# AutonomousVehicleLaboratory/vision_semantic_segmentation

Measured on AMD Instinct MI355X. Metric: fused frames/sec/GPU (1920x1080 + 120k pts) + max|dlog-odds| vs ref, higher is better.
Workload: dtype f16 hi+lo split, MX-FP4 correction passes, fp32 accumulate

## Files before the change

### vision_semantic_segmentation_amd/csrc/seg_dwpw.hip

```cpp
#include "seg_types.h"

namespace avl {
namespace {

constexpr int TM = 128;
constexpr int TN = 256;
constexpr int A_STAGE = TM * 128;
constexpr int W_STAGE = TN * 128;
constexpr int LDS_W = 0, LDS_A = 2 * W_STAGE, LDS_P = LDS_A + 2 * A_STAGE;
constexpr int P_STEP = 8 * 6 * 8 * 4;

struct DwPwArgs {
    const void* X;
    const void* X_lo;
    const void* Wc;
    const float* bc;
    float* LG;
    unsigned char* labels;
    int ncls;
    int tiles_x;
    const void* W;
    const float* bias;
    const uint32_t* dwp;
    const int* order;
// ... 189 lines not shown
                if constexpr (WSUB != 1) {
                    if (p.C_lo) {
#pragma unroll
                        for (int i = 0; i < 8; ++i) { lo[i] -= (float)(HT)lo[i]; hi[i] -= (float)(HT)hi[i]; }
                        HT* cl = static_cast<HT*>(p.C_lo) + (long long)m * p.ldc + nbase;
                        Vec8<HT>::store(cl, lo);
                        Vec8<HT>::store(cl + 8, hi);
                    }
                }
            }
        }
    }
}

constexpr int X_LDS_W = 0, X_LDS_AH = 2 * W_STAGE, X_LDS_AL = X_LDS_AH + 2 * A_STAGE, X_LDS_P = X_LDS_AL + A_STAGE;
constexpr int XP_RING = 4;
constexpr int FP_STEP = 8 * 10 * 8 * 4;

__global__ void __launch_bounds__(512) k_dwpw_x(DwPwArgs p) {
    constexpr int PSTEP = FP_STEP;
    typedef f16 HT;
    typedef typename Half16<HT>::v8 v8;
    extern __shared__ __attribute__((aligned(16))) char lds[];
    const int tid = threadIdx.x, lane = tid & 63;
    const int wave = __builtin_amdgcn_readfirstlane(tid >> 6);
    const int wm = wave >> 2, wn = wave & 3;
    const int nt = blockIdx.x % p.ntiles;
    const int bm = blockIdx.x / p.ntiles, slot = (bm & 7) * p.per_xcd + (bm >> 3);
    if (slot >= p.mtiles) return;
    dwpw_image(p);
    const int mt = p.order[slot];
    const int nk = p.K / 64;

    const uint4* psrc = reinterpret_cast<const uint4*>(p.dwp);
    uint4 pnext = make_uint4(0u, 0u, 0u, 0u);
    auto load_p = [&](int s) { if (tid < PSTEP / 16 && s < nk) pnext = psrc[s * (PSTEP / 16) + tid]; };
    auto store_p = [&](int s) { if (tid < PSTEP / 16 && s < nk) *reinterpret_cast<uint4*>(lds + X_LDS_P + (s & (XP_RING - 1)) * PSTEP + tid * 16) = pnext; };
    for (int s = 0; s < 3; ++s) { load_p(s); store_p(s); }

    const int chunk = tid & 7, r0 = tid >> 3;
    unsigned voff[2][9];
#pragma unroll
    for (int q = 0; q < 2; ++q) {
        const int m = mt * TM + r0 + q * 64;
        const int y = m / p.OW, x = m - y * p.OW;
#pragma unroll
        for (int t = 0; t < 9; ++t) {
            const int iy = y - p.pad + (t / 3) * p.dil, ix = x - p.pad + (t % 3) * p.dil;
            const bool ok = m < p.M && iy >= 0 && iy < p.H && ix >= 0 && ix < p.Wd;
            voff[q][t] = ok ? (unsigned)(((long long)iy * p.Wd + ix) * p.ldx + chunk * 8) * 2u : 0x7fffff00u;
        }
    }
    const int wchunk = tid & 7, wrow0 = tid >> 3;
    const __amdgpu_buffer_rsrc_t wrsrc = __builtin_amdgcn_make_buffer_rsrc(
        const_cast<char*>(static_cast<const char*>(p.W) + (long long)nt * TN * p.K * 4), 0, TN * p.K * 4, 0x00020000);
    int w_voff[4];
#pragma unroll
    for (int i = 0; i < 4; ++i) w_voff[i] = (wrow0 + 64 * i) * p.K * 4 + wchunk * 16;
    v4i wl[4];
    auto load_w = [&](int h) {
#pragma unroll
        for (int i = 0; i < 4; ++i) wl[i] = __builtin_amdgcn_raw_buffer_load_b128(wrsrc, w_voff[i], h * 128, 0);
    };
    auto store_w = [&](int h) {
#pragma unroll
        for (int i = 0; i < 4; ++i) {
            const int r = wrow0 + 64 * i;
            const int key = ((r >> 1) & 1) | (((r >> 4) & 3) << 1);
            *reinterpret_cast<v4i*>(lds + X_LDS_W + (h & 1) * W_STAGE + r * 128 + ((wchunk ^ key) << 4)) = wl[i];
        }
    };

    const int fr = lane & 15, kq = lane >> 4;
    int a_off[4], w_off[4], a_key[4], w_key[4];
#pragma unroll
    for (int mi = 0; mi < 4; ++mi) {
        const int row = wm * 64 + mi * 16 + fr;
        a_off[mi] = row * 128;
        a_key[mi] = row & 7;
    }
#pragma unroll
    for (int nj = 0; nj < 4; ++nj) {
        const int row = wn * 64 + (fr >> 2) * 16 + nj * 4 + (fr & 3);
        w_off[nj] = X_LDS_W + row * 128;
        w_key[nj] = ((row >> 1) & 1) | (((row >> 4) & 3) << 1);
    }
    f32x4 acc[4][4];
    {
        const int nb = nt * TN + wn * 64 + kq * 16;
#pragma unroll
        for (int nj = 0; nj < 4; ++nj) {
            const float4 b = *reinterpret_cast<const float4*>(p.bias + nb + 4 * nj);
#pragma unroll
            for (int mi = 0; mi < 4; ++mi) acc[mi][nj] = f32x4{b.x, b.y, b.z, b.w};
        }
    }

    v4i raw[2][9];
    const __amdgpu_buffer_rsrc_t xrsrc = __builtin_amdgcn_make_buffer_rsrc(const_cast<void*>(p.X), 0, (int)p.x_bytes, 0x00020000);
    auto load_taps = [&](int s, int q) {
#pragma unroll
        for (int t = 0; t < 9; ++t) raw[q][t] = __builtin_amdgcn_raw_buffer_load_b128(xrsrc, (int)voff[q][t], s * 128, 0);
    };
// ... 1 lines not shown
    auto produce_a = [&](int s, int q) {
        float o[8];
        const float* pf = reinterpret_cast<const float*>(lds + X_LDS_P + (s & (XP_RING - 1)) * PSTEP + chunk * (10 * 8 * 4));
        {
            const float4 b0 = *reinterpret_cast<const float4*>(pf + 9 * 8), b1 = *reinterpret_cast<const float4*>(pf + 9 * 8 + 4);
            o[0] = b0.x; o[1] = b0.y; o[2] = b0.z; o[3] = b0.w;
            o[4] = b1.x; o[5] = b1.y; o[6] = b1.z; o[7] = b1.w;
        }
        typedef _Float16 h2 __attribute__((ext_vector_type(2)));
#pragma unroll
        for (int t = 0; t < 9; ++t) {
            const float4 w0 = *reinterpret_cast<const float4*>(pf + t * 8), w1 = *reinterpret_cast<const float4*>(pf + t * 8 + 4);
            const float wt[8] = {w0.x, w0.y, w0.z, w0.w, w1.x, w1.y, w1.z, w1.w};
#pragma unroll
            for (int j = 0; j < 4; ++j) {
                const int u = raw[q][t][j];
                const h2 v = __builtin_bit_cast(h2, u);
                o[2 * j] = __builtin_fmaf((float)v[0], wt[2 * j], o[2 * j]);
                o[2 * j + 1] = __builtin_fmaf((float)v[1], wt[2 * j + 1], o[2 * j + 1]);
            }
        }
        float ol[8];
#pragma unroll
        for (int i = 0; i < 8; ++i) {
            o[i] = fmaxf(o[i], 0.f);
            ol[i] = o[i] - (float)(HT)o[i];
        }
        const int row = r0 + q * 64;
        const int sw = row * 128 + ((chunk ^ (row & 7)) << 4);
        Vec8<HT>::store(reinterpret_cast<HT*>(lds + X_LDS_AH + (s & 1) * A_STAGE + sw), o);
        Vec8<HT>::store(reinterpret_cast<HT*>(lds + X_LDS_AL + sw), ol);
    };

    load_taps(0, 0);
    load_taps(0, 1);
    load_w(0);
    __syncthreads();
    produce_a(0, 0);
    produce_a(0, 1);
    store_w(0);
    if (nk > 1) { load_taps(1, 0); load_taps(1, 1); }

    for (int s = 0; s < nk; ++s) {
        const bool more = s + 1 < nk, more2 = s + 2 < nk;
        asm volatile("s_waitcnt lgkmcnt(0)" ::: "memory");
        __builtin_amdgcn_s_barrier();
        load_w(2 * s + 1);
        load_p(s + 3);
#pragma unroll
        for (int kk = 0; kk < 2; ++kk) {
            v8 wa[4], ah[4], al[4];
#pragma unroll
            for (int nj = 0; nj < 4; ++nj) wa[nj] = *reinterpret_cast<const v8*>(lds + w_off[nj] + (((kk * 4 + kq) ^ w_key[nj]) << 4));
#pragma unroll
            for (int mi = 0; mi < 4; ++mi) {
                ah[mi] = *reinterpret_cast<const v8*>(lds + X_LDS_AH + (s & 1) * A_STAGE + a_off[mi] + (((kk * 4 + kq) ^ a_key[mi]) << 4));
                al[mi] = *reinterpret_cast<const v8*>(lds + X_LDS_AL + a_off[mi] + (((kk * 4 + kq) ^ a_key[mi]) << 4));
            }
#pragma unroll
            for (int mi = 0; mi < 4; ++mi)
#pragma unroll
                for (int nj = 0; nj < 4; ++nj) acc[mi][nj] = Half16<HT>::mfma(wa[nj], al[mi], acc[mi][nj]);
#pragma unroll
            for (int mi = 0; mi < 4; ++mi)
#pragma unroll
                for (int nj = 0; nj < 4; ++nj) acc[mi][nj] = Half16<HT>::mfma(wa[nj], ah[mi], acc[mi][nj]);
        }
        store_w(2 * s + 1);
        store_p(s + 3);
        asm volatile("s_waitcnt lgkmcnt(0)" ::: "memory");
        __builtin_amdgcn_s_barrier();
        if (more) load_w(2 * s + 2);
#pragma unroll
        for (int kk = 0; kk < 2; ++kk) {
            v8 wa[4], ah[4];
#pragma unroll
            for (int nj = 0; nj < 4; ++nj) wa[nj] = *reinterpret_cast<const v8*>(lds + W_STAGE + w_off[nj] + (((kk * 4 + kq) ^ w_key[nj]) << 4));
#pragma unroll
            for (int mi = 0; mi < 4; ++mi)
                ah[mi] = *reinterpret_cast<const v8*>(lds + X_LDS_AH + (s & 1) * A_STAGE + a_off[mi] + (((kk * 4 + kq) ^ a_key[mi]) << 4));
#pragma unroll
            for (int mi = 0; mi < 4; ++mi)
#pragma unroll
                for (int nj = 0; nj < 4; ++nj) acc[mi][nj] = Half16<HT>::mfma(wa[nj], ah[mi], acc[mi][nj]);
            if (more) {
                produce_a(s + 1, kk);
                if (more2) load_taps(s + 2, kk);
            }
        }
        if (more) store_w(2 * s + 2);
    }

    const int nbase = nt * TN + wn * 64 + kq * 16;
    if (nbase + 16 <= p.N) {
#pragma unroll
        for (int mi = 0; mi < 4; ++mi) {
            const int m = mt * TM + wm * 64 + mi * 16 + fr;
            if (m < p.M) {
                float lo[8], hi[8];
#pragma unroll
                for (int nj = 0; nj < 2; ++nj)
#pragma unroll
                    for (int r = 0; r < 4; ++r) {
                        lo[nj * 4 + r] = fmaxf(acc[mi][nj][r], 0.f);
                        hi[nj * 4 + r] = fmaxf(acc[mi][2 + nj][r], 0.f);
                    }
                HT* cp = static_cast<HT*>(p.C) + (long long)m * p.ldc + nbase;
                Vec8<HT>::store(cp, lo);
                Vec8<HT>::store(cp + 8, hi);
                if (p.C_lo) {
#pragma unroll
                    for (int i = 0; i < 8; ++i) { lo[i] -= (float)(HT)lo[i]; hi[i] -= (float)(HT)hi[i]; }
                    HT* cl = static_cast<HT*>(p.C_lo) + (long long)m * p.ldc + nbase;
                    Vec8<HT>::store(cl, lo);
                    Vec8<HT>::store(cl + 8, hi);
                }
            }
        }
    }
}

int launch_dwpw_x(const DwPwArgs& a, hipStream_t s) {
    constexpr int lds_bytes = X_LDS_P + XP_RING * FP_STEP;
    static_assert(lds_bytes <= 160 * 1024, "k_dwpw_x LDS");
// ... 409 lines not shown
```

### vision_semantic_segmentation_amd/csrc/seg_gconv_mfma.hip

```cpp
#include <cstring>

#include "seg_types.h"

namespace avl {
namespace {

constexpr int TW = 32;
constexpr int CC = 64;

template <typename HT>
struct GconvArgs {
    const HT* in;
    const HT* in_lo;
    const HT* w;
    const float* bias;
    HT* out;
    HT* out_lo;
    char* oq[2];
    char* os[2];
    long long o_srows;
    int H, W, in_ld, OH, OW, out_ld, C;
    int stride, dil;
    int th;
    int tiles_x, tiles_y, cchunks;
    int comb;
    int nsp, nslots;
    int walk;
    int tile_bytes;
    int tw_magic;
    const char* w4;
    const char* w4s;
    const char* xq[2];
    const char* xs[2];
    long long x_srows;
    int dephase;
};

constexpr int ROWS_PITCH = 40, ROWS_IN_TH = 6;
constexpr int ROWS_TILE_BYTES = ROWS_IN_TH * ROWS_PITCH * 128 + 4 * 4096 + 2 * 1024;
static_assert(2 * ROWS_TILE_BYTES <= 160 * 1024 && ROWS_PITCH % 8 == 0 && ROWS_PITCH >= TW + 2, "two row-aligned tile buffers fit the CU's LDS");

template <typename T>
__device__ __forceinline__ T lds_load(unsigned byte_addr) {
    return *(const __attribute__((address_space(3))) T*)(size_t)byte_addr;
}

template <typename HT, int WS, int NJ, bool XS = false, bool ROWS = false>
__global__ void __launch_bounds__(512) k_gconv_mfma(GconvArgs<HT> p) {
    static_assert(!XS || WS == 1, "a split input goes with split weights");
    static_assert(!ROWS || (WS == 2 && NJ == 2), "the row-aligned tile is the MX variant's four-row tile");
    typedef typename Half16<HT>::v8 v8;
    extern __shared__ __attribute__((aligned(16))) char lds[];
    const int tid = threadIdx.x, lane = tid & 63;
    const int wave = __builtin_amdgcn_readfirstlane(tid >> 6);
    {
        const long long ipix = (long long)p.H * p.W, opix = (long long)p.OH * p.OW;
        p.in = image_base(p.in, ipix, p.in_ld);
        p.in_lo = image_base(p.in_lo, ipix, p.in_ld);
        p.out = image_base(p.out, opix, p.out_ld);
        p.out_lo = image_base(p.out_lo, opix, p.out_ld);
#pragma unroll
        for (int pl = 0; pl < 2; ++pl) {
            p.oq[pl] = image_base(p.oq[pl], opix, p.C / 2);
            p.os[pl] = image_base(p.os[pl], opix, 8);
            p.xq[pl] = image_base(p.xq[pl], ipix, p.C / 2);
            p.xs[pl] = image_base(p.xs[pl], ipix, 8);
        }
    }
    int bid = blockIdx.x;
    {
        const int nwg = gridDim.x, xcd = bid & 7, local = bid >> 3, q = nwg >> 3, r = nwg & 7;
        bid = (xcd < r ? xcd * (q + 1) : r * (q + 1) + (xcd - r) * q) + local;
    }
    const int cchunk = bid % p.cchunks, slot = bid / p.cchunks;
    const int s = ROWS ? 1 : p.stride;
    const int d = ROWS ? 1 : p.comb ? 1 : p.dil;
    const int step = p.comb ? p.dil : 1;
    const int th = ROWS ? 4 : p.th;
    const int in_th = ROWS ? ROWS_IN_TH : (th - 1) * s + 2 * d + 1, in_tw = ROWS ? ROWS_PITCH : (TW - 1) * s + 2 * d + 1;
    const int tile_bytes = ROWS ? ROWS_TILE_BYTES : p.tile_bytes;
    const int c0 = cchunk * CC;
    const int npix = in_th * in_tw;
    const int ngroups = (npix + 7) >> 3;
    const unsigned lds0 = lds_addr(lds);
    const int n64 = (npix + 63) >> 6;
    const int QBASE = ngroups * 1024, QT = n64 * 1024, SBASE = QBASE + 4 * QT, ST = n64 * 256;
    const bool has_lo = WS == 2 && p.xq[1] != nullptr;
    const int LOBASE = ngroups * 1024;
// ... 18 lines not shown
            const int cy = min(max(iy, 0), p.H - 1), cx = min(max(ix, 0), p.W - 1);
            const unsigned voff = ((unsigned)(cy * p.W + cx) * (unsigned)p.in_ld + ((cphys ^ (pix & 7)) << 3)) * (unsigned)sizeof(HT);
            glds16_saddr(p.in + c0, voff, lds0 + buf * tile_bytes + gi * 1024);
            if constexpr (XS) glds16_saddr(p.in_lo + c0, voff, lds0 + buf * tile_bytes + LOBASE + gi * 1024);
            oob |= outside << it;
        }
        if constexpr (WS == 2) {
            const int pwbits = has_lo ? 2 : 1;
            it = 16;
            for (int item = wave; item < (n64 << pwbits); item += 8, ++it) {
                const int pw = item & ((1 << pwbits) - 1), gq = item >> pwbits, w = pw & 1, pl = pw >> 1;
                const int pix = gq * 64 + lane;
                const int ly = (pix * p.tw_magic) >> 16, lx = pix - ly * in_tw;
                const int iy = iy0 + ly * step, ix = ix0 + lx * step;
                const unsigned outside = (unsigned)(pix >= npix) | (unsigned)((unsigned)iy >= (unsigned)p.H) | (unsigned)((unsigned)ix >= (unsigned)p.W);
                const int cy = min(max(iy, 0), p.H - 1), cx = min(max(ix, 0), p.W - 1);
                glds16_saddr(xq0 + pl * xq_delta + c0 / 2 + w * 16, (unsigned)(cy * p.W + cx) * (unsigned)(p.C / 2),
                             lds0 + buf * tile_bytes + QBASE + (pl * 2 + w) * QT + gq * 1024);
                oob |= outside << it;
            }
            for (int item = wave; item < (n64 << (pwbits - 1)); item += 8) {
                const int pl = item & ((1 << (pwbits - 1)) - 1), gq = item >> (pwbits - 1);
                const int pix = gq * 64 + lane;
                const int ly = (pix * p.tw_magic) >> 16, lx = pix - ly * in_tw;
                const int cy = min(max(iy0 + ly * step, 0), p.H - 1), cx = min(max(ix0 + lx * step, 0), p.W - 1);
                glds4_saddr(xs0 + pl * xs_delta + ((long long)(c0 >> 8) * p.x_srows) * 8 + ((c0 >> 5) & 4), (unsigned)(cy * p.W + cx) * 8u,
                            lds0 + buf * tile_bytes + SBASE + pl * ST + gq * 256);
            }
        }
        return oob;
    };
    const int col_lane = (lane >> 3) * step;
    const unsigned swz_lane = (unsigned)(((lane & 7) ^ (lane >> 3)) << 3) * (unsigned)sizeof(HT);
    auto stage_rows = [&](int ty, int tx, int ry, int rx, int buf) -> unsigned {
        const int iy0 = ry + (ty * 4 - 1) * step, ix0 = rx + (tx * TW - 1) * step;
        const unsigned dst = lds0 + buf * ROWS_TILE_BYTES;
        const unsigned ld_bytes = (unsigned)p.in_ld * (unsigned)sizeof(HT);
        unsigned oob = 0;
#pragma unroll
        for (int it = 0; it < 4; ++it) {
            const int gi = wave + 8 * it;
            if (gi < ROWS_IN_TH * (ROWS_PITCH / 8)) {
                const int ly = gi / (ROWS_PITCH / 8), g8 = gi - ly * (ROWS_PITCH / 8);
                const int iy = iy0 + ly * step, ix = ix0 + g8 * 8 * step + col_lane;
                const unsigned outside = (unsigned)((unsigned)iy >= (unsigned)p.H) | (unsigned)((unsigned)ix >= (unsigned)p.W);
                const int cy = min(max(iy, 0), p.H - 1), cx = min(max(ix, 0), p.W - 1);
                const unsigned voff = (unsigned)(cy * p.W) * ld_bytes + __umul24((unsigned)cx, ld_bytes) + swz_lane;
                glds16_saddr(p.in + c0, voff, dst + gi * 1024);
                oob |= outside << it;
            }
        }
        const int pwbits = has_lo ? 2 : 1;
        int it = 16;
        for (int item = wave; item < (4 << pwbits); item += 8, ++it) {
            const int pw = item & ((1 << pwbits) - 1), gq = item >> pwbits, w = pw & 1, pl = pw >> 1;
            const int pix = gq * 64 + lane;
            const int ly = (pix * 1639) >> 16, lx = pix - ly * ROWS_PITCH;
            const int iy = __mul24(ly, step) + iy0, ix = __mul24(lx, step) + ix0;
            const unsigned outside = (unsigned)(pix >= ROWS_IN_TH * ROWS_PITCH) | (unsigned)((unsigned)iy >= (unsigned)p.H) | (unsigned)((unsigned)ix >= (unsigned)p.W);
            const int cy = min(max(iy, 0), p.H - 1), cx = min(max(ix, 0), p.W - 1);
            glds16_saddr(xq0 + pl * xq_delta + c0 / 2 + w * 16, (__umul24((unsigned)cy, (unsigned)p.W) + (unsigned)cx) * (unsigned)(p.C / 2),
                         dst + QBASE + (pl * 2 + w) * QT + gq * 1024);
            oob |= outside << it;
        }
        for (int item = wave; item < (4 << (pwbits - 1)); item += 8) {
            const int pl = item & ((1 << (pwbits - 1)) - 1), gq = item >> (pwbits - 1);
            const int pix = gq * 64 + lane;
            const int ly = (pix * 1639) >> 16, lx = pix - ly * ROWS_PITCH;
            const int cy = min(max(__mul24(ly, step) + iy0, 0), p.H - 1), cx = min(max(__mul24(lx, step) + ix0, 0), p.W - 1);
            glds4_saddr(xs0 + pl * xs_delta + ((long long)(c0 >> 8) * p.x_srows) * 8 + ((c0 >> 5) & 4), (__umul24((unsigned)cy, (unsigned)p.W) + (unsigned)cx) * 8u,
                        dst + SBASE + pl * ST + gq * 256);
        }
        return oob;
    };
    const int per = (p.nsp + p.nslots - 1) / p.nslots;
    const int sp_step = ROWS || p.walk ? 1 : p.nslots, sp_end = ROWS || p.walk ? min(p.nsp, (slot + 1) * per) : p.nsp;
    int sp = ROWS || p.walk ? slot * per : slot, buf = 0;
    int ty = 0, tx = 0, ry = 0, rx = 0, nty = 0, ntx = 0, nry = 0, nrx = 0;
    auto advance = [&](int& y, int& x, int& cy, int& cx) {
        if (++y == p.tiles_y) {
            y = 0;
            if (++x == p.tiles_x) {
                x = 0;
                if (++cx == p.dil) { cx = 0; ++cy; }
            }
        }
    };
    if constexpr (ROWS) {
        ty = sp % p.tiles_y;
        const int r1 = sp / p.tiles_y;
        tx = r1 % p.tiles_x;
        const int cmb = r1 / p.tiles_x;
        ry = p.comb ? cmb / p.dil : 0; rx = p.comb ? cmb % p.dil : 0;
        nty = ty; ntx = tx; nry = ry; nrx = rx;
        advance(nty, ntx, nry, nrx);
    }
    auto stage_tile = [&](bool next, int b) -> unsigned {
        if constexpr (ROWS) return next ? stage_rows(nty, ntx, nry, nrx, b) : stage_rows(ty, tx, ry, rx, b);
        else return stage(next ? sp + sp_step : sp, b);
    };
    unsigned oob = sp < sp_end ? stage_tile(false, 0) : 0u;

    const int win = wave & 1;
    const int part = wave >> 1;
    const int fr = lane & 15, kq = lane >> 4;
    constexpr int NT = WS == 1 ? 18 : 9;
    v8 wf[2][NT];
    {
        const HT* wp = p.w + (long long)(cchunk * 2 + win) * (2 * NT * 16 * 32);
#pragma unroll
        for (int nj = 0; nj < 2; ++nj)
#pragma unroll
            for (int t = 0; t < NT; ++t)
                wf[nj][t] = *reinterpret_cast<const v8*>(wp + ((nj * NT + t) * 16 + fr) * 32 + kq * 8);
    }
    int4 w4[WS == 2 ? 2 : 1][2][3];
    unsigned w4sc[3] = {0u, 0u, 0u};
    if constexpr (WS == 2) {
        const long long widx = cchunk * 2 + win;
        const char* w4p = p.w4 + widx * (2 * 2 * 3 * 64 * 16) + lane * 16;
#pragma unroll
        for (int nj = 0; nj < 2; ++nj)
#pragma unroll
            for (int pr = 0; pr < 2; ++pr)
#pragma unroll
                for (int g = 0; g < 3; ++g) w4[nj][pr][g] = *reinterpret_cast<const int4*>(w4p + ((nj * 2 + pr) * 3 + g) * (64 * 16));
        const unsigned* sp = reinterpret_cast<const unsigned*>(p.w4s + widx * (64 * 12) + lane * 12);
        w4sc[0] = sp[0]; w4sc[1] = sp[1]; w4sc[2] = sp[2];
    }
    const int ssel = 8 * (((c0 >> 5) & 3) + win);
    const int cbase = c0 + win * 32 + kq * 8;
// ... 29 lines not shown
    zero_oob(oob, 0);
    __syncthreads();

    constexpr bool HOIST = NJ <= 2 && WS != 2;
    int toff[HOIST ? NJ : 1][9];
    if constexpr (HOIST) {
#pragma unroll
        for (int j = 0; j < NJ; ++j) {
            const int st = part + 4 * j;
            const int sy = st >> 1, sx = (st & 1) * 16 + fr;
#pragma unroll
            for (int t = 0; t < 9; ++t) {
                const int pix = (sy * s + (t / 3) * d) * in_tw + sx * s + (t % 3) * d;
                toff[j][t] = pix * 128 + ((chunk_in ^ (pix & 7)) << 4);
            }
        }
    }
    unsigned a_addr[3] = {0u, 0u, 0u}, q_addr[3] = {0u, 0u, 0u}, s_addr[3] = {0u, 0u, 0u};
    if constexpr (ROWS) {
        const int row0 = part >> 1, sx = (part & 1) * 16 + fr;
#pragma unroll
        for (int c = 0; c < 3; ++c)
            a_addr[c] = lds0 + (row0 * ROWS_PITCH + sx + c) * 128 + ((chunk_in ^ ((sx + c) & 7)) << 4);
#pragma unroll
        for (int g = 0; g < 3; ++g) {
            const int t = min(4 * g + kq, 8);
            const int pix = (row0 + t / 3) * ROWS_PITCH + sx + t % 3;
            q_addr[g] = lds0 + QBASE + win * QT + pix * 16;
            s_addr[g] = lds0 + SBASE + pix * 4 + (ssel >> 3);
        }
    }
    const unsigned o_ld = (unsigned)p.out_ld, q_ld = (unsigned)(p.C / 2);
    const unsigned sc_lane = (unsigned)(cbase >> 8) * (unsigned)p.o_srows * 8u + (unsigned)((cbase >> 5) & 7);

    for (; sp < sp_end; sp += sp_step, buf ^= 1) {
        const bool late_stage = NJ >= 2 && wave >= 4 && p.dephase;
        oob = 0u;
        if (!late_stage && sp + sp_step < sp_end) oob = stage_tile(true, buf ^ 1);
        const char* tile = lds + buf * tile_bytes;
        f32x4 acc[NJ][2];
#pragma unroll
        for (int j = 0; j < NJ; ++j) {
            if (NJ >= 2 && j == NJ / 2 && late_stage && sp + sp_step < sp_end) oob = stage_tile(true, buf ^ 1);
            v8 a[9];
            if constexpr (ROWS) {
#pragma unroll
                for (int t = 0; t < 9; ++t) a[t] = lds_load<v8>(a_addr[t % 3] + (2 * j + t / 3) * (ROWS_PITCH * 128));
            } else if constexpr (HOIST) {
#pragma unroll
                for (int t = 0; t < 9; ++t) a[t] = *reinterpret_cast<const v8*>(tile + toff[j][t]);
            } else {
                const int st = part + 4 * j;
                int frv = fr;
                asm volatile("" : "+v"(frv));
                const int sy = st >> 1, sx = (st & 1) * 16 + frv;
#pragma unroll
                for (int t = 0; t < 9; ++t) {
                    const int pix = (sy * s + (t / 3) * d) * in_tw + sx * s + (t % 3) * d;
                    a[t] = *reinterpret_cast<const v8*>(tile + pix * 128 + ((chunk_in ^ (pix & 7)) << 4));
                }
            }
            f32x4 acc0 = bias0, acc1 = bias1;
            if constexpr (WS == 2) {
                typedef int v8i __attribute__((ext_vector_type(8)));
                const int st2 = part + 4 * j;
                const int sy2 = st2 >> 1, sx2 = (st2 & 1) * 16 + fr;
// ... 51 lines not shown
#pragma unroll
                        for (int t = 0; t < 9; ++t) a[t] = *reinterpret_cast<const v8*>(tile + LOBASE + toff[j][t]);
                    } else {
                        const int st = part + 4 * j;
                        int frv = fr;
                        asm volatile("" : "+v"(frv));
                        const int sy = st >> 1, sx = (st & 1) * 16 + frv;
#pragma unroll
                        for (int t = 0; t < 9; ++t) {
                            const int pix = (sy * s + (t / 3) * d) * in_tw + sx * s + (t % 3) * d;
                            a[t] = *reinterpret_cast<const v8*>(tile + LOBASE + pix * 128 + ((chunk_in ^ (pix & 7)) << 4));
                        }
                    }
#pragma unroll
                    for (int t = 0; t < 9; ++t) {
                        acc0 = Half16<HT>::mfma(wf[0][t], a[t], acc0);
                        acc1 = Half16<HT>::mfma(wf[1][t], a[t], acc1);
                    }
                }
            }
            acc[j][0] = acc0; acc[j][1] = acc1;
            __builtin_amdgcn_sched_barrier(0);
        }
        asm volatile("s_waitcnt vmcnt(0)" ::: "memory");
        zero_oob(oob, buf ^ 1);

        int etx = tx, ety = ty, ery = ry, erx = rx;
        if constexpr (!ROWS) {
            int cmb;
            if (p.walk) { ety = sp % p.tiles_y; const int r1 = sp / p.tiles_y; etx = r1 % p.tiles_x; cmb = r1 / p.tiles_x; }
            else { etx = sp % p.tiles_x; const int r1 = sp / p.tiles_x; ety = r1 % p.tiles_y; cmb = r1 / p.tiles_y; }
            ery = p.comb ? cmb / p.dil : 0; erx = p.comb ? cmb % p.dil : 0;
        }
        const int oy0 = ety * th, ox0 = etx * TW;
#pragma unroll
        for (int j = 0; j < NJ; ++j) {
            const int st = part + 4 * j;
            const int sy = st >> 1, sx = (st & 1) * 16 + fr;
            const int oy = ery + (oy0 + sy) * step, ox = erx + (ox0 + sx) * step;
            const bool live = oy < p.OH && ox < p.OW;
            const unsigned pix = live ? (unsigned)oy * (unsigned)p.OW + (unsigned)ox : 0u;
            float v[8];
#pragma unroll
            for (int r = 0; r < 4; ++r) {
                v[r] = fmaxf(acc[j][0][r], 0.f);
                v[4 + r] = fmaxf(acc[j][1][r], 0.f);
            }
            if constexpr (WS == 0) {
                if (live) Vec8<HT>::store(p.out + (pix * o_ld + (unsigned)cbase), v);
            } else {
                typedef typename Half16<HT>::v8 h8;
                typedef HT h2 __attribute__((ext_vector_type(2)));
                typedef unsigned u4 __attribute__((ext_vector_type(4)));
                u4 hpk;
#pragma unroll
                for (int r = 0; r < 4; ++r) {
                    const h2 t = {(HT)v[2 * r], (HT)v[2 * r + 1]};
                    hpk[r] = __builtin_bit_cast(unsigned, t);
                }
                const h8 hv = __builtin_bit_cast(h8, hpk);
                if (live) *reinterpret_cast<h8*>(p.out + (pix * o_ld + (unsigned)cbase)) = hv;
                float lo[8];
#pragma unroll
                for (int r = 0; r < 8; ++r) {
                    const float h = (float)hv[r];
                    lo[r] = v[r] - h;
                    v[r] = h;
                }
                if (p.out_lo) {
                    h8 lv;
#pragma unroll
                    for (int r = 0; r < 8; ++r) lv[r] = (HT)lo[r];
                    if (live) *reinterpret_cast<h8*>(p.out_lo + (pix * o_ld + (unsigned)cbase)) = lv;
#pragma unroll
                    for (int r = 0; r < 8; ++r) lo[r] = (float)lv[r];
                }
#pragma unroll
                for (int pl = 0; pl < 2; ++pl) {
                    if (p.oq[pl] == nullptr) continue;
                    const float* src = pl == 0 ? v : lo;
                    float amax = 0.f;
#pragma unroll
                    for (int r = 0; r < 8; ++r) amax = fmaxf(amax, fabsf(src[r]));
                    {
                        const unsigned ab = __float_as_uint(amax);
                        const auto r16 = __builtin_amdgcn_permlane16_swap(ab, ab, false, false);
                        const unsigned m16 = max(r16[0], r16[1]);
                        const auto r32 = __builtin_amdgcn_permlane32_swap(m16, m16, false, false);
                        amax = __uint_as_float(max(r32[0], r32[1]));
                    }
                    const unsigned sbyte = mx_fp4_scale_byte(amax);
                    const float scale = __uint_as_float(sbyte << 23);
                    unsigned pk = 0u;
                    pk = __builtin_amdgcn_cvt_scalef32_pk_fp4_f32(pk, src[0], src[1], scale, 0);
                    pk = __builtin_amdgcn_cvt_scalef32_pk_fp4_f32(pk, src[2], src[3], scale, 1);
                    pk = __builtin_amdgcn_cvt_scalef32_pk_fp4_f32(pk, src[4], src[5], scale, 2);
                    pk = __builtin_amdgcn_cvt_scalef32_pk_fp4_f32(pk, src[6], src[7], scale, 3);
                    if (live) {
                        *reinterpret_cast<unsigned*>(p.oq[pl] + (pix * q_ld + (unsigned)(cbase / 2))) = pk;
                        if (kq == 0) p.os[pl][sc_lane + pix * 8u] = (char)sbyte;
                    }
                }
            }
            __builtin_amdgcn_sched_barrier(0);
        }
        if constexpr (ROWS) {
            ty = nty; tx = ntx; ry = nry; rx = nrx;
            advance(nty, ntx, nry, nrx);
            const unsigned flip = buf ? (unsigned)-ROWS_TILE_BYTES : (unsigned)ROWS_TILE_BYTES;
#pragma unroll
            for (int i = 0; i < 3; ++i) { a_addr[i] += flip; q_addr[i] += flip; s_addr[i] += flip; }
        }
        __syncthreads();
    }
}

}

int gconv_mfma_lds_bytes(int stride, int dil, int& th) {
    th = stride == 1 ? 8 : 4;
    const int in_th = (th - 1) * stride + 2 * dil + 1, in_tw = (TW - 1) * stride + 2 * dil + 1;
    return ((in_th * in_tw + 7) / 8) * 1024;
}

static int gconv_tile_bytes(int stride, int dil, int th, bool mx = false, bool xs = false) {
    const int in_th = (th - 1) * stride + 2 * dil + 1, in_tw = (TW - 1) * stride + 2 * dil + 1;
    const int npix = in_th * in_tw, n64 = (npix + 63) / 64;
    return ((npix + 7) / 8) * 1024 * (xs ? 2 : 1) + (mx ? 4 * n64 * 1024 + 2 * n64 * 256 : 0);
}

static int device_cus() {
    static int n = 0;
    if (n == 0) {
        int dev = 0;
        hipDeviceProp_t prop;
        if (hipGetDevice(&dev) == hipSuccess && hipGetDeviceProperties(&prop, dev) == hipSuccess) n = prop.multiProcessorCount;
        if (n <= 0) n = 256;
    }
    return n;
}

// ... 25 lines not shown
template <typename HT, int WS, bool XS = false>
int launch_gconv_typed(const avl_seg_op& op, hipStream_t s) {
    GconvArgs<HT> a;
    a.in = static_cast<const HT*>(op.in);
    a.in_lo = static_cast<const HT*>(op.in_lo);
    a.w = static_cast<const HT*>(op.weight);
    a.bias = op.bias;
    a.out = static_cast<HT*>(op.out);
    a.out_lo = static_cast<HT*>(op.out_lo);
    a.oq[0] = a.oq[1] = a.os[0] = a.os[1] = nullptr;
    a.o_srows = op.out_rows;
    if (op.out_mx) {
        const auto o = mx_bundle(op.out_mx, op.out_rows, op.out_c);
        a.oq[0] = o.q[0]; a.os[0] = o.s[0];
        if (op.out_lo || (op.mx_flags & AVL_MX_OUT_LO)) { a.oq[1] = o.q[1]; a.os[1] = o.s[1]; }
    }
    a.H = op.in_h; a.W = op.in_w; a.in_ld = op.in_ld; a.OH = op.out_h; a.OW = op.out_w; a.out_ld = op.out_ld; a.C = op.in_c;
    a.stride = op.stride; a.dil = op.dil;
    a.comb = (op.stride == 1 && op.dil > 1 && op.pad == op.dil) ? 1 : 0;
    a.th = gconv_pick_th(op, a.comb, device_cus(), &a.nsp, &a.nslots);
    AVL_REQUIRE(a.th > 0, "grouped conv: no tile height fits two LDS buffers");
    const bool rows = WS == 2 && !XS && op.w_split == 2 && op.stride == 1 && (op.dil == 1 || a.comb) && a.th == 4 && op.in_lo == nullptr;
    a.tile_bytes = rows ? ROWS_TILE_BYTES : gconv_tile_bytes(op.stride, a.comb ? 1 : op.dil, a.th, WS == 2, XS);
    a.w4 = a.w4s = a.xq[0] = a.xq[1] = a.xs[0] = a.xs[1] = nullptr;
    a.x_srows = op.in_rows;
    if (WS == 2) {
        const long long nwin = op.in_c / 32;
        a.w4 = static_cast<const char*>(op.w_mx);
        a.w4s = a.w4 + nwin * (2 * 2 * 3 * 64 * 16);
        const auto x = mx_bundle(op.in_mx, op.in_rows, op.in_c);
        a.xq[0] = x.q[0]; a.xs[0] = x.s[0];
        if (op.mx_flags & AVL_MX_IN_LO) { a.xq[1] = x.q[1]; a.xs[1] = x.s[1]; }
    }
    {
        const int d = a.comb ? 1 : op.dil;
        const int in_th = (a.th - 1) * op.stride + 2 * d + 1, in_tw = (TW - 1) * op.stride + 2 * d + 1;
        a.tw_magic = (65536 + in_tw - 1) / in_tw;
        for (int pix = 0; pix < ((in_th * in_tw + 63) / 64) * 64; ++pix)
            AVL_REQUIRE(((pix * a.tw_magic) >> 16) == pix / in_tw, "grouped conv: tile %d x %d too large for the reciprocal division", in_th, in_tw);
    }
    const int gh = a.comb ? (op.out_h + op.dil - 1) / op.dil : op.out_h, gw = a.comb ? (op.out_w + op.dil - 1) / op.dil : op.out_w;
    a.tiles_x = (gw + TW - 1) / TW;
    a.tiles_y = (gh + a.th - 1) / a.th;
    a.cchunks = op.in_c / CC;
#define AVL_GCONV_LAUNCH(NJ, ROWS)                                                                                                    \
    do {                                                                                                                              \
        AVL_HIP_CHECK(hipFuncSetAttribute(reinterpret_cast<const void*>(&k_gconv_mfma<HT, WS, NJ, XS, ROWS>), hipFuncAttributeMaxDynamicSharedMemorySize, 160 * 1024)); \
        hipLaunchKernelGGL((k_gconv_mfma<HT, WS, NJ, XS, ROWS>), dim3(a.nslots * a.cchunks, 1, op_batch(op)), dim3(512), 2 * a.tile_bytes, s, a); \
    } while (0)
    a.dephase = 1;
    a.walk = 1;
    if (a.th == 8) {
        if constexpr (WS != 2 && !XS) AVL_GCONV_LAUNCH(4, false);
        else return avl::set_error(AVL_E_ARG, "MX / split-input grouped conv: tile height 8 is not built");
    }
    else if (a.th == 4) {
        if constexpr (WS == 2 && !XS) {
            if (rows) AVL_GCONV_LAUNCH(2, true);
            else AVL_GCONV_LAUNCH(2, false);
        } else AVL_GCONV_LAUNCH(2, false);
    }
    else AVL_GCONV_LAUNCH(1, false);
#undef AVL_GCONV_LAUNCH
    AVL_LAUNCH_CHECK();
    return AVL_OK;
}
// ... 34 lines not shown
```

Measured before the change: 242.7.

## Stream weights and dw params straight to LDS via global-load-to-LDS DMA

Replaces the register-staged buffer loads plus LDS stores for the pointwise weight tiles and depthwise parameter ring with direct global-to-LDS loads, folding the XOR swizzle into the per-lane global offset. The aim is to free VGPRs and VALU/LDS-store instructions and let weight loads land in LDS without a register round trip. The tap-load schedule is made unconditional, so the last iterations reload already-used taps, and explicit vmcnt waits are added to order DMA completion against the barriers. The hard-coded vmcnt counts tie correctness to the exact number of outstanding loads.

```diff
diff --git a/vision_semantic_segmentation_amd/csrc/seg_dwpw.hip b/vision_semantic_segmentation_amd/csrc/seg_dwpw.hip
--- a/vision_semantic_segmentation_amd/csrc/seg_dwpw.hip
+++ b/vision_semantic_segmentation_amd/csrc/seg_dwpw.hip
@@ -245,11 +245,12 @@
     const int mt = p.order[slot];
     const int nk = p.K / 64;
 
-    const uint4* psrc = reinterpret_cast<const uint4*>(p.dwp);
-    uint4 pnext = make_uint4(0u, 0u, 0u, 0u);
-    auto load_p = [&](int s) { if (tid < PSTEP / 16 && s < nk) pnext = psrc[s * (PSTEP / 16) + tid]; };
-    auto store_p = [&](int s) { if (tid < PSTEP / 16 && s < nk) *reinterpret_cast<uint4*>(lds + X_LDS_P + (s & (XP_RING - 1)) * PSTEP + tid * 16) = pnext; };
-    for (int s = 0; s < 3; ++s) { load_p(s); store_p(s); }
+    const unsigned lds0 = lds_addr(lds);
+    auto dma_p = [&](int s) {
+        if (tid < PSTEP / 16 && s < nk)
+            glds16_saddr(reinterpret_cast<const char*>(p.dwp) + s * PSTEP, (unsigned)tid * 16u, lds0 + X_LDS_P + (s & (XP_RING - 1)) * PSTEP + wave * 1024);
+    };
+    for (int s = 0; s < 3; ++s) dma_p(s);
 
     const int chunk = tid & 7, r0 = tid >> 3;
     unsigned voff[2][9];
@@ -264,24 +265,17 @@
             voff[q][t] = ok ? (unsigned)(((long long)iy * p.Wd + ix) * p.ldx + chunk * 8) * 2u : 0x7fffff00u;
         }
     }
-    const int wchunk = tid & 7, wrow0 = tid >> 3;
-    const __amdgpu_buffer_rsrc_t wrsrc = __builtin_amdgcn_make_buffer_rsrc(
-        const_cast<char*>(static_cast<const char*>(p.W) + (long long)nt * TN * p.K * 4), 0, TN * p.K * 4, 0x00020000);
-    int w_voff[4];
-#pragma unroll
-    for (int i = 0; i < 4; ++i) w_voff[i] = (wrow0 + 64 * i) * p.K * 4 + wchunk * 16;
-    v4i wl[4];
-    auto load_w = [&](int h) {
-#pragma unroll
-        for (int i = 0; i < 4; ++i) wl[i] = __builtin_amdgcn_raw_buffer_load_b128(wrsrc, w_voff[i], h * 128, 0);
-    };
-    auto store_w = [&](int h) {
-#pragma unroll
-        for (int i = 0; i < 4; ++i) {
-            const int r = wrow0 + 64 * i;
-            const int key = ((r >> 1) & 1) | (((r >> 4) & 3) << 1);
-            *reinterpret_cast<v4i*>(lds + X_LDS_W + (h & 1) * W_STAGE + r * 128 + ((wchunk ^ key) << 4)) = wl[i];
-        }
+    const char* wbase = static_cast<const char*>(p.W) + (long long)nt * TN * p.K * 4;
+    unsigned w_voff;
+    {
+        const int r = wave * 8 + (lane >> 3);
+        const int key = ((r >> 1) & 1) | (((r >> 4) & 3) << 1);
+        w_voff = (unsigned)(r * p.K * 4 + (((lane & 7) ^ key) << 4));
+    }
+    const int w_rows64 = 64 * p.K * 4;
+    auto dma_w = [&](int h) {
+#pragma unroll
+        for (int i = 0; i < 4; ++i) glds16_saddr(wbase + h * 128 + i * w_rows64, w_voff, lds0 + X_LDS_W + (h & 1) * W_STAGE + i * 8192 + wave * 1024);
     };
 
     const int fr = lane & 15, kq = lane >> 4;
@@ -349,21 +343,22 @@
         Vec8<HT>::store(reinterpret_cast<HT*>(lds + X_LDS_AL + sw), ol);
     };
 
+    dma_w(0);
     load_taps(0, 0);
     load_taps(0, 1);
-    load_w(0);
+    asm volatile("s_waitcnt vmcnt(18)" ::: "memory");
     __syncthreads();
     produce_a(0, 0);
     produce_a(0, 1);
-    store_w(0);
     if (nk > 1) { load_taps(1, 0); load_taps(1, 1); }
 
     for (int s = 0; s < nk; ++s) {
-        const bool more = s + 1 < nk, more2 = s + 2 < nk;
+        const bool more = s + 1 < nk;
+        const int s_taps = s + 2 < nk ? s + 2 : s;
         asm volatile("s_waitcnt lgkmcnt(0)" ::: "memory");
         __builtin_amdgcn_s_barrier();
-        load_w(2 * s + 1);
-        load_p(s + 3);
+        dma_p(s + 3);
+        dma_w(2 * s + 1);
 #pragma unroll
         for (int kk = 0; kk < 2; ++kk) {
             v8 wa[4], ah[4], al[4];
@@ -383,11 +378,11 @@
 #pragma unroll
                 for (int nj = 0; nj < 4; ++nj) acc[mi][nj] = Half16<HT>::mfma(wa[nj], ah[mi], acc[mi][nj]);
         }
-        store_w(2 * s + 1);
-        store_p(s + 3);
+        __builtin_amdgcn_sched_barrier(0);
+        asm volatile("s_waitcnt vmcnt(0)" ::: "memory");
         asm volatile("s_waitcnt lgkmcnt(0)" ::: "memory");
         __builtin_amdgcn_s_barrier();
-        if (more) load_w(2 * s + 2);
+        if (more) dma_w(2 * s + 2);
 #pragma unroll
         for (int kk = 0; kk < 2; ++kk) {
             v8 wa[4], ah[4];
@@ -400,13 +395,12 @@
             for (int mi = 0; mi < 4; ++mi)
 #pragma unroll
                 for (int nj = 0; nj < 4; ++nj) acc[mi][nj] = Half16<HT>::mfma(wa[nj], ah[mi], acc[mi][nj]);
-            if (more) {
-                produce_a(s + 1, kk);
-                if (more2) load_taps(s + 2, kk);
-            }
-        }
-        if (more) store_w(2 * s + 2);
-    }
+            if (more) produce_a(s + 1, kk);
+            load_taps(s_taps, kk);
+        }
+        asm volatile("s_waitcnt vmcnt(18)" ::: "memory");
+    }
+    asm volatile("s_waitcnt vmcnt(0)" ::: "memory");
 
     const int nbase = nt * TN + wn * 64 + kq * 16;
     if (nbase + 16 <= p.N) {
```

After: 244.9 (median of 6 runs). About the same (+0.9%).

## Incrementally advance row-tile staging and epilogue addresses with buffer stores

Applied to the files above, without the earlier changes.

For the row-aligned MX grouped-conv variant, staging offsets are kept in registers and advanced by four rows when the next tile is directly below, instead of being recomputed with clamps each tile. The epilogue writes the f16 hi/lo and FP4 outputs through raw buffer stores, using out-of-range offsets in place of per-lane live checks, and reloads output pointers from the kernarg segment to save registers. Batch and plane offsets are folded into 32-bit offsets, which requires new host checks on bundle layout and size limits. This trims address arithmetic and register pressure, at the cost of relying on buffer out-of-bounds behaviour and fixed layout assumptions.

```diff
diff --git a/vision_semantic_segmentation_amd/csrc/seg_gconv_mfma.hip b/vision_semantic_segmentation_amd/csrc/seg_gconv_mfma.hip
--- a/vision_semantic_segmentation_amd/csrc/seg_gconv_mfma.hip
+++ b/vision_semantic_segmentation_amd/csrc/seg_gconv_mfma.hip
@@ -53,7 +53,7 @@
     extern __shared__ __attribute__((aligned(16))) char lds[];
     const int tid = threadIdx.x, lane = tid & 63;
     const int wave = __builtin_amdgcn_readfirstlane(tid >> 6);
-    {
+    if constexpr (!ROWS) {
         const long long ipix = (long long)p.H * p.W, opix = (long long)p.OH * p.OW;
         p.in = image_base(p.in, ipix, p.in_ld);
         p.in_lo = image_base(p.in_lo, ipix, p.in_ld);
@@ -138,44 +138,94 @@
     };
     const int col_lane = (lane >> 3) * step;
     const unsigned swz_lane = (unsigned)(((lane & 7) ^ (lane >> 3)) << 3) * (unsigned)sizeof(HT);
-    auto stage_rows = [&](int ty, int tx, int ry, int rx, int buf) -> unsigned {
+    const int wave0 = wave;
+    unsigned r_off[7] = {0u, 0u, 0u, 0u, 0u, 0u, 0u};
+    unsigned oob_col = 0u;
+    const unsigned zin = ROWS ? blockIdx.z * (unsigned)(p.H * p.W) : 0u;
+    const unsigned x_pb = ROWS ? (unsigned)mx_plane_bytes(p.x_srows, p.C) : 0u, x_ps = ROWS ? x_pb + (unsigned)mx_scale_bytes(p.x_srows, p.C) : 0u;
+    auto stage_rows = [&](bool add, int ty, int tx, int ry, int rx, int buf) -> unsigned {
+        const unsigned dst = __builtin_amdgcn_readfirstlane(lds0 + buf * ROWS_TILE_BYTES);
+        const unsigned ld_bytes = (unsigned)p.in_ld * (unsigned)sizeof(HT), q_bytes = (unsigned)(p.C / 2);
+        const int pwbits = has_lo ? 2 : 1;
+        int wave = wave0;
+        asm volatile("" : "+s"(wave));
+        const bool has_g3 = wave < ROWS_IN_TH * (ROWS_PITCH / 8) - 24, has_sc = has_lo || wave < 4;
+        if (add) {
+            const unsigned row4 = (unsigned)(4 * step * p.W);
+#pragma unroll
+            for (int it = 0; it < 4; ++it) {
+                const int gi = wave + 8 * it;
+                if (it < 3 || has_g3) {
+                    r_off[it] += row4 * ld_bytes;
+                    glds16_saddr(p.in, r_off[it], dst + gi * 1024);
+                }
+            }
+#pragma unroll
+            for (int k = 0; k < 2; ++k) {
+                const int item = wave + 8 * k;
+                if (k == 0 || has_lo) {
+                    const int pw = item & ((1 << pwbits) - 1), gq = item >> pwbits;
+                    r_off[4 + k] += row4 * q_bytes;
+                    glds16_saddr(p.xq[0], r_off[4 + k], dst + QBASE + pw * QT + gq * 1024);
+                }
+            }
+            if (has_sc) {
+                const int pl = wave & ((1 << (pwbits - 1)) - 1), gq = wave >> (pwbits - 1);
+                r_off[6] += row4 * 8u;
+                glds4_saddr(p.xq[0], r_off[6], dst + SBASE + pl * ST + gq * 256);
+            }
+            return oob_col;
+        }
         const int iy0 = ry + (ty * 4 - 1) * step, ix0 = rx + (tx * TW - 1) * step;
-        const unsigned dst = lds0 + buf * ROWS_TILE_BYTES;
-        const unsigned ld_bytes = (unsigned)p.in_ld * (unsigned)sizeof(HT);
         unsigned oob = 0;
+        oob_col = 0u;
+        int lane = tid & 63;
+        asm volatile("" : "+v"(lane));
+        const int col_lane = (lane >> 3) * step;
+        const unsigned swz_lane = (unsigned)(((lane & 7) ^ (lane >> 3)) << 3) * (unsigned)sizeof(HT);
 #pragma unroll
         for (int it = 0; it < 4; ++it) {
             const int gi = wave + 8 * it;
-            if (gi < ROWS_IN_TH * (ROWS_PITCH / 8)) {
+            if (it < 3 || has_g3) {
                 const int ly = gi / (ROWS_PITCH / 8), g8 = gi - ly * (ROWS_PITCH / 8);
                 const int iy = iy0 + ly * step, ix = ix0 + g8 * 8 * step + col_lane;
-                const unsigned outside = (unsigned)((unsigned)iy >= (unsigned)p.H) | (unsigned)((unsigned)ix >= (unsigned)p.W);
+                const unsigned out_col = (unsigned)((unsigned)ix >= (unsigned)p.W);
+                const unsigned outside = (unsigned)((unsigned)iy >= (unsigned)p.H) | out_col;
                 const int cy = min(max(iy, 0), p.H - 1), cx = min(max(ix, 0), p.W - 1);
-                const unsigned voff = (unsigned)(cy * p.W) * ld_bytes + __umul24((unsigned)cx, ld_bytes) + swz_lane;
-                glds16_saddr(p.in + c0, voff, dst + gi * 1024);
+                r_off[it] = (unsigned)(iy * p.W) * ld_bytes + __umul24((unsigned)cx, ld_bytes) + swz_lane + (zin * (unsigned)p.in_ld + (unsigned)c0) * (unsigned)sizeof(HT);
+                const unsigned voff = r_off[it] + (unsigned)((cy - iy) * p.W) * ld_bytes;
+                glds16_saddr(p.in, voff, dst + gi * 1024);
                 oob |= outside << it;
-            }
-        }
-        const int pwbits = has_lo ? 2 : 1;
-        int it = 16;
-        for (int item = wave; item < (4 << pwbits); item += 8, ++it) {
-            const int pw = item & ((1 << pwbits) - 1), gq = item >> pwbits, w = pw & 1, pl = pw >> 1;
+                oob_col |= out_col << it;
+            }
+        }
+#pragma unroll
+        for (int k = 0; k < 2; ++k) {
+            const int item = wave + 8 * k;
+            if (k == 0 || has_lo) {
+                const int pw = item & ((1 << pwbits) - 1), gq = item >> pwbits, w = pw & 1, pl = pw >> 1;
+                const int pix = gq * 64 + lane;
+                const int ly = min((pix * 1639) >> 16, ROWS_IN_TH - 1), lx = pix - ((pix * 1639) >> 16) * ROWS_PITCH;
+                const int iy = __mul24(ly, step) + iy0, ix = __mul24(lx, step) + ix0;
+                const unsigned out_col = (unsigned)(pix >= ROWS_IN_TH * ROWS_PITCH) | (unsigned)((unsigned)ix >= (unsigned)p.W);
+                const unsigned outside = out_col | (unsigned)((unsigned)iy >= (unsigned)p.H);
+                const int cy = min(max(iy, 0), p.H - 1), cx = min(max(ix, 0), p.W - 1);
+                const unsigned base = (unsigned)pl * x_ps + zin * q_bytes + (unsigned)(c0 / 2 + w * 16);
+                r_off[4 + k] = (unsigned)(iy * p.W + cx) * q_bytes + base;
+                glds16_saddr(p.xq[0], (__umul24((unsigned)cy, (unsigned)p.W) + (unsigned)cx) * q_bytes + base, dst + QBASE + pw * QT + gq * 1024);
+                oob |= outside << (16 + k);
+                oob_col |= out_col << (16 + k);
+            }
+        }
+        if (has_sc) {
+            const int pl = wave & ((1 << (pwbits - 1)) - 1), gq = wave >> (pwbits - 1);
             const int pix = gq * 64 + lane;
-            const int ly = (pix * 1639) >> 16, lx = pix - ly * ROWS_PITCH;
-            const int iy = __mul24(ly, step) + iy0, ix = __mul24(lx, step) + ix0;
-            const unsigned outside = (unsigned)(pix >= ROWS_IN_TH * ROWS_PITCH) | (unsigned)((unsigned)iy >= (unsigned)p.H) | (unsigned)((unsigned)ix >= (unsigned)p.W);
-            const int cy = min(max(iy, 0), p.H - 1), cx = min(max(ix, 0), p.W - 1);
-            glds16_saddr(xq0 + pl * xq_delta + c0 / 2 + w * 16, (__umul24((unsigned)cy, (unsigned)p.W) + (unsigned)cx) * (unsigned)(p.C / 2),
-                         dst + QBASE + (pl * 2 + w) * QT + gq * 1024);
-            oob |= outside << it;
-        }
-        for (int item = wave; item < (4 << (pwbits - 1)); item += 8) {
-            const int pl = item & ((1 << (pwbits - 1)) - 1), gq = item >> (pwbits - 1);
-            const int pix = gq * 64 + lane;
-            const int ly = (pix * 1639) >> 16, lx = pix - ly * ROWS_PITCH;
-            const int cy = min(max(__mul24(ly, step) + iy0, 0), p.H - 1), cx = min(max(__mul24(lx, step) + ix0, 0), p.W - 1);
-            glds4_saddr(xs0 + pl * xs_delta + ((long long)(c0 >> 8) * p.x_srows) * 8 + ((c0 >> 5) & 4), (__umul24((unsigned)cy, (unsigned)p.W) + (unsigned)cx) * 8u,
-                        dst + SBASE + pl * ST + gq * 256);
+            const int ly = min((pix * 1639) >> 16, ROWS_IN_TH - 1), lx = pix - ((pix * 1639) >> 16) * ROWS_PITCH;
+            const int iy = __mul24(ly, step) + iy0;
+            const int cy = min(max(iy, 0), p.H - 1), cx = min(max(__mul24(lx, step) + ix0, 0), p.W - 1);
+            const unsigned base = x_pb + (unsigned)pl * x_ps + (unsigned)(c0 >> 8) * (unsigned)p.x_srows * 8u + (unsigned)((c0 >> 5) & 4) + zin * 8u;
+            r_off[6] = (unsigned)(iy * p.W + cx) * 8u + base;
+            glds4_saddr(p.xq[0], (__umul24((unsigned)cy, (unsigned)p.W) + (unsigned)cx) * 8u + base, dst + SBASE + pl * ST + gq * 256);
         }
         return oob;
     };
@@ -201,8 +251,11 @@
         nty = ty; ntx = tx; nry = ry; nrx = rx;
         advance(nty, ntx, nry, nrx);
     }
+    auto steps_down = [&](int y, int cy) { return y != 0 && cy + (4 * y + 4) * step < p.H; };
+    bool cur_add = false, next_add = false;
+    if constexpr (ROWS) next_add = steps_down(nty, nry);
     auto stage_tile = [&](bool next, int b) -> unsigned {
-        if constexpr (ROWS) return next ? stage_rows(nty, ntx, nry, nrx, b) : stage_rows(ty, tx, ry, rx, b);
+        if constexpr (ROWS) return next ? stage_rows(next_add, nty, ntx, nry, nrx, b) : stage_rows(false, ty, tx, ry, rx, b);
         else return stage(next ? sp + sp_step : sp, b);
     };
     unsigned oob = sp < sp_end ? stage_tile(false, 0) : 0u;
@@ -298,6 +351,11 @@
     }
     const unsigned o_ld = (unsigned)p.out_ld, q_ld = (unsigned)(p.C / 2);
     const unsigned sc_lane = (unsigned)(cbase >> 8) * (unsigned)p.o_srows * 8u + (unsigned)((cbase >> 5) & 7);
+    unsigned e_f0 = 0x80000000u, e_s0 = 0x80000000u;
+    unsigned e_f1 = 0x80000000u, e_s1 = 0x80000000u;
+    const unsigned zout = ROWS ? blockIdx.z * (unsigned)(p.OH * p.OW) : 0u;
+    const unsigned o_bytes = ROWS ? gridDim.z * (unsigned)(p.OH * p.OW) * o_ld * (unsigned)sizeof(HT) : 0u;
+    const unsigned o_pb = ROWS ? (unsigned)mx_plane_bytes(p.o_srows, p.C) : 0u, o_ps = ROWS ? o_pb + (unsigned)mx_scale_bytes(p.o_srows, p.C) : 0u;
 
     for (; sp < sp_end; sp += sp_step, buf ^= 1) {
         const bool late_stage = NJ >= 2 && wave >= 4 && p.dephase;
@@ -415,6 +473,32 @@
             else { etx = sp % p.tiles_x; const int r1 = sp / p.tiles_x; ety = r1 % p.tiles_y; cmb = r1 / p.tiles_y; }
             ery = p.comb ? cmb / p.dil : 0; erx = p.comb ? cmb % p.dil : 0;
         }
+        if constexpr (ROWS) {
+            {
+                auto ka = __builtin_amdgcn_kernarg_segment_ptr();
+                asm volatile("" : "+s"(ka));
+                const GconvArgs<HT>* ea = (const GconvArgs<HT>*)ka;
+                p.out = ea->out; p.out_lo = ea->out_lo; p.oq[0] = ea->oq[0]; p.oq[1] = ea->oq[1];
+            }
+            const unsigned e_row = (unsigned)(step * p.OW);
+            if (cur_add) {
+                e_f0 += 4u * e_row * o_ld * (unsigned)sizeof(HT);
+                e_s0 += 4u * e_row * 8u;
+            } else {
+                int l = tid & 63;
+                asm volatile("" : "+v"(l));
+                const int lfr = l & 15, lkq = l >> 4, lcbase = c0 + win * 32 + lkq * 8;
+                const int oy = ery + (ety * 4 + (part >> 1)) * step, ox = erx + (etx * TW + (part & 1) * 16 + lfr) * step;
+                const bool live = oy < p.OH && ox < p.OW;
+                const unsigned pix = zout + (unsigned)oy * (unsigned)p.OW + (unsigned)ox;
+                const unsigned lsc = (unsigned)(lcbase >> 8) * (unsigned)p.o_srows * 8u + (unsigned)((lcbase >> 5) & 7);
+                e_f0 = live ? (pix * o_ld + (unsigned)lcbase) * (unsigned)sizeof(HT) : 0x80000000u;
+                e_s0 = live && lkq == 0 ? o_pb + lsc + pix * 8u : 0x80000000u;
+            }
+            const unsigned dead1 = ery + (ety * 4 + (part >> 1) + 2) * step < p.OH ? 0u : 0x80000000u;
+            e_f1 = max(e_f0 + 2u * e_row * o_ld * (unsigned)sizeof(HT), dead1);
+            e_s1 = max(e_s0 + 2u * e_row * 8u, dead1);
+        }
         const int oy0 = ety * th, ox0 = etx * TW;
 #pragma unroll
         for (int j = 0; j < NJ; ++j) {
@@ -442,7 +526,8 @@
                     hpk[r] = __builtin_bit_cast(unsigned, t);
                 }
                 const h8 hv = __builtin_bit_cast(h8, hpk);
-                if (live) *reinterpret_cast<h8*>(p.out + (pix * o_ld + (unsigned)cbase)) = hv;
+                if constexpr (ROWS) __builtin_amdgcn_raw_buffer_store_b128(hpk, __builtin_amdgcn_make_buffer_rsrc(p.out, 0, (int)o_bytes, 0x00020000), (int)(j ? e_f1 : e_f0), 0, 0);
+                else if (live) *reinterpret_cast<h8*>(p.out + (pix * o_ld + (unsigned)cbase)) = hv;
                 float lo[8];
 #pragma unroll
                 for (int r = 0; r < 8; ++r) {
@@ -454,7 +539,9 @@
                     h8 lv;
 #pragma unroll
                     for (int r = 0; r < 8; ++r) lv[r] = (HT)lo[r];
-                    if (live) *reinterpret_cast<h8*>(p.out_lo + (pix * o_ld + (unsigned)cbase)) = lv;
+                    if constexpr (ROWS)
+                        __builtin_amdgcn_raw_buffer_store_b128(__builtin_bit_cast(u4, lv), __builtin_amdgcn_make_buffer_rsrc(p.out_lo, 0, (int)o_bytes, 0x00020000), (int)(j ? e_f1 : e_f0), 0, 0);
+                    else if (live) *reinterpret_cast<h8*>(p.out_lo + (pix * o_ld + (unsigned)cbase)) = lv;
 #pragma unroll
                     for (int r = 0; r < 8; ++r) lo[r] = (float)lv[r];
                 }
@@ -479,7 +566,11 @@
                     pk = __builtin_amdgcn_cvt_scalef32_pk_fp4_f32(pk, src[2], src[3], scale, 1);
                     pk = __builtin_amdgcn_cvt_scalef32_pk_fp4_f32(pk, src[4], src[5], scale, 2);
                     pk = __builtin_amdgcn_cvt_scalef32_pk_fp4_f32(pk, src[6], src[7], scale, 3);
-                    if (live) {
+                    if constexpr (ROWS) {
+                        const __amdgpu_buffer_rsrc_t q_rsrc = __builtin_amdgcn_make_buffer_rsrc(p.oq[0] + (pl ? o_ps : 0u), 0, (int)o_ps, 0x00020000);
+                        __builtin_amdgcn_raw_buffer_store_b32(pk, q_rsrc, (int)(j ? e_f1 : e_f0) >> 2, 0, 0);
+                        __builtin_amdgcn_raw_buffer_store_b8((unsigned char)sbyte, q_rsrc, (int)(j ? e_s1 : e_s0), 0, 0);
+                    } else if (live) {
                         *reinterpret_cast<unsigned*>(p.oq[pl] + (pix * q_ld + (unsigned)(cbase / 2))) = pk;
                         if (kq == 0) p.os[pl][sc_lane + pix * 8u] = (char)sbyte;
                     }
@@ -490,6 +581,8 @@
         if constexpr (ROWS) {
             ty = nty; tx = ntx; ry = nry; rx = nrx;
             advance(nty, ntx, nry, nrx);
+            cur_add = next_add;
+            next_add = steps_down(nty, nry);
             const unsigned flip = buf ? (unsigned)-ROWS_TILE_BYTES : (unsigned)ROWS_TILE_BYTES;
 #pragma unroll
             for (int i = 0; i < 3; ++i) { a_addr[i] += flip; q_addr[i] += flip; s_addr[i] += flip; }
@@ -581,6 +674,14 @@
         a.xq[0] = x.q[0]; a.xs[0] = x.s[0];
         if (op.mx_flags & AVL_MX_IN_LO) { a.xq[1] = x.q[1]; a.xs[1] = x.s[1]; }
     }
+    if (rows) {
+        const long long xp = mx_plane_bytes(op.in_rows, op.in_c), xps = xp + mx_scale_bytes(op.in_rows, op.in_c);
+        const long long opl = mx_plane_bytes(op.out_rows, op.out_c), ops = opl + mx_scale_bytes(op.out_rows, op.out_c);
+        AVL_REQUIRE(a.xs[0] == a.xq[0] + xp && (!a.xq[1] || (a.xq[1] == a.xq[0] + xps && a.xs[1] == a.xq[1] + xp)) && 2 * xps < (1LL << 32),
+                    "MX grouped conv: the input bundle is not laid out as mx_bundle_at states, or exceeds 4 GB");
+        AVL_REQUIRE(!a.oq[0] || (a.os[0] == a.oq[0] + opl && (!a.oq[1] || (a.oq[1] == a.oq[0] + ops && a.os[1] == a.oq[1] + opl)) && ops < (1LL << 31) && op.out_ld == op.out_c),
+                    "MX grouped conv: the output bundle is not laid out as mx_bundle_at states, or a half of it exceeds 2 GB");
+    }
     {
         const int d = a.comb ? 1 : op.dil;
         const int in_th = (a.th - 1) * op.stride + 2 * d + 1, in_tw = (TW - 1) * op.stride + 2 * d + 1;
```

Result: no change. 239.2 before, 239.5 after, median of 2 (+0.1%).
